# Hawkeye-FineGrained/Hawkeye

Hardware: AMD Instinct MI355X
Metric: images/sec (train fwd+bwd) BCNN VGG-16 448^2 bs64 (higher is better)
Workload: dtype f32; 1 GPU; BCNN_S2: VGG-16 448x448, per-GPU batch 64, 200 classes, SGD momentum 0.9, CE label_smoothing 0.1, full train step; global_batch=64, parallelism=dp1, memory_format=channels_last

## Files before the change

### hawkeye_amd/csrc/conv_fwd.hip

```cpp
#include "hk_common.h"
#include "hk_split_bf16.h"
#include <hk_mfma_bf16.h>
#include "../../include/hawkeye_hip.h"

namespace hk {

constexpr int CF_CO = 64;
constexpr int CF_R = 4;
constexpr int CF_SW = 32;
constexpr int CF_CK = 32;
constexpr int CF_PIX = 80;
constexpr int CF_HW = CF_SW + 2;
constexpr int CF_HPIX = (CF_R + 2) * CF_HW;
constexpr int CF_XPLANE = CF_HPIX * CF_PIX;
constexpr int CF_WPLANE = CF_CO * CF_PIX;
constexpr int CF_WTAP = 3 * CF_WPLANE;
constexpr int CF_LDS = 3 * CF_XPLANE + 2 * CF_WTAP;
constexpr int CF_XF4 = CF_HPIX * (CF_CK / 4);
constexpr int CF_XU = (CF_XF4 + 255) / 256;
constexpr int CF_FLUSH = 3;

constexpr int CF_MF_32 = 0, CF_MF_16 = 1;
constexpr int CF16_PIX = 64;
constexpr int CF16_XPLANE = CF_HPIX * CF16_PIX;
constexpr int CF16_WPLANE = CF_CO * CF16_PIX;
constexpr int CF16_WTAP = 3 * CF16_WPLANE;
constexpr int CF16_LDS = 3 * CF16_XPLANE + 2 * CF16_WTAP;
__host__ __device__ constexpr int cf16_off(int row, int kg) { return row * CF16_PIX + ((kg ^ ((row >> 1) & 2)) << 4); }
constexpr int CF_B128_GROUPS[4][16] = {{0, 1, 2, 3, 12, 13, 14, 15, 20, 21, 22, 23, 24, 25, 26, 27},
                                       {4, 5, 6, 7, 8, 9, 10, 11, 16, 17, 18, 19, 28, 29, 30, 31},
                                       {32, 33, 34, 35, 44, 45, 46, 47, 52, 53, 54, 55, 56, 57, 58, 59},
                                       {36, 37, 38, 39, 40, 41, 42, 43, 48, 49, 50, 51, 60, 61, 62, 63}};
constexpr bool cf16_group_conflict_free(int g) {
    for (int base = 0; base + 16 <= CF_HPIX; ++base) {
        unsigned seen = 0;
        for (int i = 0; i < 16; ++i) {
            const int lane = CF_B128_GROUPS[g][i], slot = (cf16_off(base + (lane & 15), lane >> 4) >> 4) & 15;
            if ((seen >> slot) & 1u) return false;
            seen |= 1u << slot;
        }
    }
    return true;
}
static_assert(cf16_group_conflict_free(0) && cf16_group_conflict_free(1) && cf16_group_conflict_free(2) && cf16_group_conflict_free(3),
              "every ds_read_b128 lane group of a CF_MF_16 fragment reads 16 different slots");
static_assert(cf16_off(16, 1) == cf16_off(0, 1) + 16 * CF16_PIX && cf16_off(35, 2) == cf16_off(3, 2) + 32 * CF16_PIX,
              "rows 16 and 32 further on are a constant offset away");
static_assert(CF16_WTAP <= CF_WTAP && CF16_WTAP == 3 * 256 * 16, "the workspace holds either image; a weight tile is three loads a thread");

template <int MF>
__global__ __launch_bounds__(256) void conv3x3_wsplit_kernel(const float* __restrict__ w, char* __restrict__ ws, int M, int K,
                                                             int transposed, long long total) {
    const long long i = (long long)blockIdx.x * 256 + threadIdx.x;
    if (i >= total) return;
    const int nchunk = K / CF_CK;
    constexpr int NQ = MF == CF_MF_32 ? 10 : 8;
    const int q = (int)(i % NQ);
    long long r = i / NQ;
    const int co = (int)(r % CF_CO);
    r /= CF_CO;
    const int tap = (int)(r % 9);
    const int chunk = (int)((r / 9) % nchunk), cot = (int)((r / 9) / nchunk);
    const long long m = (long long)cot * CF_CO + co, k0 = (long long)chunk * CF_CK + 4 * q;
    f32x4 v = {0.f, 0.f, 0.f, 0.f};
    if (q < 8) {
        if (!transposed) {
            v = *reinterpret_cast<const f32x4*>(w + (m * 9 + tap) * K + k0);
        } else {
#pragma unroll
            for (int e = 0; e < 4; ++e) v[e] = w[((k0 + e) * 9 + (8 - tap)) * M + m];
        }
    }
    bf16x4 p[3];
    wrs_split(v, p);
    if (MF == CF_MF_32) {
        char* d = ws + (size_t)r * CF_WTAP + co * CF_PIX + q * 8;
#pragma unroll
        for (int s = 0; s < 3; ++s) *reinterpret_cast<bf16x4*>(d + s * CF_WPLANE) = p[s];
    } else {
        char* d = ws + (size_t)r * CF16_WTAP + cf16_off(co, q >> 1) + (q & 1) * 8;
#pragma unroll
        for (int s = 0; s < 3; ++s) *reinterpret_cast<bf16x4*>(d + s * CF16_WPLANE) = p[s];
    }
}

__device__ __forceinline__ bf16x8 cf_frag(const char* p) {
#if defined(__HIP_DEVICE_COMPILE__)
    return *(const __attribute__((address_space(3))) bf16x8*)p;
#else
    bf16x8 f;
    __builtin_memcpy(&f, p, 16);
    return f;
#endif
}

constexpr int CF_EPI_NONE = 0, CF_EPI_RELU = 1, CF_EPI_POOL = 2, CF_EPI_MASK = 3;
constexpr int CF_PARK = CF_CO + 4;
constexpr int CF_DB_RPG = 128;
static_assert(CF_R * CF_SW * CF_PARK * 4 <= CF_LDS, "the parked tile fits the LDS of the main loop");

__device__ __forceinline__ f32x4 cf_relu4(f32x4 v) {
    f32x4 r;
#pragma unroll
    for (int t = 0; t < 4; ++t) r[t] = v[t] < 0.f ? 0.f : v[t];
    return r;
}
__device__ __forceinline__ unsigned cf_sign4(f32x4 r) {
    return (!(r[0] <= 0.f) ? 1u : 0u) | (!(r[1] <= 0.f) ? 2u : 0u) | (!(r[2] <= 0.f) ? 4u : 0u) | (!(r[3] <= 0.f) ? 8u : 0u);
}

template <int EPI>
__device__ __forceinline__ void cf16_epilogue(const f32x4 (&acc4)[4][2], const f32x4 (&sum4)[4][2], float* ldsf, float* __restrict__ y, int H,
                                              int W, int Cout, long long n, int r0, int c0, int cot, int tile, int wave, int tid, int l15,
                                              int kg, const float* __restrict__ bias, uint8_t* __restrict__ mk,
                                              double* __restrict__ part) {
    const int row = r0 + wave, c4 = Cout / 4;
    bool live[2];
    long long pix[2];
    f32x4 v[4][2];
#pragma unroll
    for (int pb = 0; pb < 2; ++pb) {
        const int col = c0 + 16 * pb + l15;
        live[pb] = row < H && col < W;
        pix[pb] = (n * H + row) * W + col;
#pragma unroll
        for (int cb = 0; cb < 4; ++cb) v[cb][pb] = sum4[cb][pb] + acc4[cb][pb];
    }
    if (EPI == CF_EPI_RELU || EPI == CF_EPI_POOL) {
        const f32x4* b4 = reinterpret_cast<const f32x4*>(bias + cot * CF_CO + 4 * kg);
#pragma unroll
        for (int cb = 0; cb < 4; ++cb) {
            const f32x4 b = b4[4 * cb];
#pragma unroll
            for (int pb = 0; pb < 2; ++pb) v[cb][pb] = cf_relu4(v[cb][pb] + b);
        }
    }
    if (EPI == CF_EPI_MASK) {
        typedef unsigned u32x4 __attribute__((ext_vector_type(4)));
#pragma unroll
        for (int pb = 0; pb < 2; ++pb) {
            u32x4 mb = {0u, 0u, 0u, 0u};
            if (live[pb]) mb = *reinterpret_cast<const u32x4*>(mk + pix[pb] * c4 + cot * (CF_CO / 4));
#pragma unroll
            for (int cb = 0; cb < 4; ++cb) {
                const unsigned bits = mb[cb] >> (8 * kg);
#pragma unroll
                for (int e = 0; e < 4; ++e) v[cb][pb][e] = ((bits >> e) & 1u) != 0u ? v[cb][pb][e] : 0.f;
            }
        }
    }
    if (EPI != CF_EPI_POOL) {
#pragma unroll
        for (int pb = 0; pb < 2; ++pb)
            if (live[pb]) {
                float* yp = y + pix[pb] * Cout + cot * CF_CO + 4 * kg;
#pragma unroll
                for (int cb = 0; cb < 4; ++cb) *reinterpret_cast<f32x4*>(yp + 16 * cb) = v[cb][pb];
            }
    }
    if (EPI == CF_EPI_RELU) {
        if (mk) {
#pragma unroll
            for (int pb = 0; pb < 2; ++pb) {
                unsigned own = 0;
#pragma unroll
                for (int cb = 0; cb < 4; ++cb) own |= cf_sign4(v[cb][pb]) << (8 * cb);
                unsigned m4 = 0;
#pragma unroll
                for (int j = 0; j < 4; ++j) m4 |= ((__shfl(own, l15 + 16 * j) >> (8 * kg)) & 0xffu) << (8 * j);
                if (live[pb]) *reinterpret_cast<unsigned*>(mk + pix[pb] * c4 + cot * (CF_CO / 4) + 4 * kg) = m4;
            }
        }
    }
    if (EPI == CF_EPI_POOL) {
        float* park = ldsf;
#pragma unroll
        for (int pb = 0; pb < 2; ++pb) {
            float* mine = park + (wave * CF_SW + 16 * pb + l15) * CF_PARK + 4 * kg;
#pragma unroll
            for (int cb = 0; cb < 4; ++cb) *reinterpret_cast<f32x4*>(mine + 16 * cb) = v[cb][pb];
        }
    }
    if (EPI == CF_EPI_MASK) {
        double s[16];
#pragma unroll
        for (int cb = 0; cb < 4; ++cb)
#pragma unroll
            for (int e = 0; e < 4; ++e) s[4 * cb + e] = (double)v[cb][0][e] + (double)v[cb][1][e];
#pragma unroll
        for (int d = 8; d >= 1; d >>= 1) {
            const bool up = (l15 & d) != 0;
#pragma unroll
            for (int i = 0; i < d; ++i) {
                const double send = up ? s[i] : s[i + d], keep = up ? s[i + d] : s[i];
                s[i] = keep + __shfl_xor(send, d);
            }
        }
        double* red = reinterpret_cast<double*>(ldsf);
        red[wave * CF_CO + 16 * (l15 >> 2) + 4 * kg + (l15 & 3)] = s[0];
        __syncthreads();
        if (tid < CF_CO)
            part[(long long)tile * Cout + cot * CF_CO + tid] = ((red[tid] + red[CF_CO + tid]) + red[2 * CF_CO + tid]) + red[3 * CF_CO + tid];
    }
}

template <int EPI, int MF>
__global__ __launch_bounds__(256, 2) void conv3x3_split_kernel(const float* __restrict__ x, const char* __restrict__ ws,
                                                               float* __restrict__ y, int H, int W, int Cin, int Cout, int nstrips,
                                                               int nrb, int ntiles, const float* __restrict__ bias,
                                                               uint8_t* __restrict__ mk, double* __restrict__ part) {
    constexpr bool M32 = MF == CF_MF_32;
    constexpr int XPLANE = M32 ? CF_XPLANE : CF16_XPLANE, WTAP = M32 ? CF_WTAP : CF16_WTAP;
    HK_DYN_LDS16(ldsf);
    char* xs = reinterpret_cast<char*>(ldsf);
    char* wb = xs + 3 * XPLANE;
    const int tid = threadIdx.x, lane = tid & 63, l31 = lane & 31, hf = lane >> 5;
    const int l15 = lane & 15, kg = lane >> 4;
    const int wave = __builtin_amdgcn_readfirstlane(tid >> 6);
    const int ncot = Cout / CF_CO, nchunk = Cin / CF_CK, total = nchunk * 9;
    int tile, cot;
    if (!xcd_map(blockIdx.x, ntiles, ncot, tile, cot)) return;
    const int strip = tile % nstrips, tr = tile / nstrips;
    const int rb = tr % nrb;
    const long long n = tr / nrb;
    const int c0 = strip * CF_SW, r0 = rb * CF_R;
    const float* xi = x + n * H * W * Cin;
    const char* wt = ws + (size_t)cot * total * WTAP + tid * 16;

    long long xoff[CF_XU];
    unsigned xok = 0;
#pragma unroll
    for (int u = 0; u < CF_XU; ++u) {
        const int idx = tid + 256 * u;
        const bool in = idx < CF_XF4;
        const int p = in ? idx >> 3 : 0, hr = p / CF_HW, hc = p - hr * CF_HW;
        const int row = r0 - 1 + hr, col = c0 - 1 + hc;
        if (in && row >= 0 && row < H && col >= 0 && col < W) xok |= 1u << u;
        const int rc = row < 0 ? 0 : (row < H ? row : H - 1), cc = col < 0 ? 0 : (col < W ? col : W - 1);
        xoff[u] = ((long long)rc * W + cc) * Cin + 4 * (idx & 7);
    }
    const int xdst = M32 ? (tid >> 3) * CF_PIX + (tid & 7) * 8 : cf16_off(tid >> 3, (tid & 7) >> 1) + (tid & 1) * 8;
    const int w3 = tid < 192 ? 3 * 4096 : 0;
    constexpr int NVW = M32 ? 4 : 3;

    f32x4 vx[CF_XU], vw[NVW];
    auto load_x = [&](int chunk) {
        const float* b = xi + chunk * CF_CK;
#pragma unroll
        for (int u = 0; u < CF_XU; ++u) HK_LOAD16_ASYNC(vx[u], b + xoff[u]);
    };
    auto load_w = [&](int it) {
        const char* b = wt + (size_t)it * WTAP;
#pragma unroll
        for (int u = 0; u < 3; ++u) HK_LOAD16_ASYNC(vw[u], reinterpret_cast<const float*>(b + 4096 * u));
        if constexpr (M32) {
            HK_LOAD16_ASYNC(vw[3], reinterpret_cast<const float*>(b + w3));
        }
    };
    auto store_x = [&]() {
        const f32x4 zero = {0.f, 0.f, 0.f, 0.f};
#pragma unroll
        for (int u = 0; u < CF_XU; ++u) {
            if (tid + 256 * u < CF_XF4) {
                bf16x4 p[3];
                wrs_split(((xok >> u) & 1) ? vx[u] : zero, p);
#pragma unroll
                for (int s = 0; s < 3; ++s) *reinterpret_cast<bf16x4*>(xs + s * XPLANE + xdst + u * 32 * (M32 ? CF_PIX : CF16_PIX)) = p[s];
            }
        }
    };
    auto store_w = [&](int buf) {
        char* d = wb + buf * WTAP + tid * 16;
#pragma unroll
        for (int u = 0; u < 3; ++u) *reinterpret_cast<f32x4*>(d + 4096 * u) = vw[u];
        if constexpr (M32) {
            if (tid < 192) *reinterpret_cast<f32x4*>(d + 3 * 4096) = vw[3];
        }
    };

    f32x16 acc[2], sum[2];
    f32x4 acc4[4][2], sum4[4][2];
    if constexpr (M32) {
#pragma unroll
        for (int cb = 0; cb < 2; ++cb)
#pragma unroll
            for (int i = 0; i < 16; ++i) acc[cb][i] = sum[cb][i] = 0.f;
    } else {
#pragma unroll
        for (int cb = 0; cb < 4; ++cb)
#pragma unroll
            for (int pb = 0; pb < 2; ++pb)
#pragma unroll
                for (int e = 0; e < 4; ++e) acc4[cb][pb][e] = sum4[cb][pb][e] = 0.f;
    }

    load_w(0);
    load_x(0);
    __builtin_amdgcn_s_waitcnt(HK_VMCNT_IMM(0));
#pragma unroll
    for (int u = 0; u < NVW; ++u) HK_PIN_LOADED(vw[u]);
#pragma unroll
    for (int u = 0; u < CF_XU; ++u) HK_PIN_LOADED(vx[u]);
    store_x();
    store_w(0);
    __syncthreads();

    const int aoff = l31 * CF_PIX + hf * 16;
    const int boff = (wave * CF_HW + l31) * CF_PIX + hf * 16;
    int since = 0;
    for (int chunk = 0; chunk < nchunk; ++chunk) {
        const bool more = chunk + 1 < nchunk;
#pragma unroll
        for (int tap = 0; tap < 9; ++tap) {
            const int it = chunk * 9 + tap;
            load_w(it + 1 < total ? it + 1 : it);
            if (tap == 5) load_x(more ? chunk + 1 : chunk);
            if constexpr (M32) {
            const char* A = wb + (it & 1) * CF_WTAP + aoff;
            const char* B = xs + boff + ((tap / 3) * CF_HW + tap % 3) * CF_PIX;
            bf16x8 a[2][2][3], b[2][3];
#pragma unroll
            for (int ks = 0; ks < 2; ++ks)
#pragma unroll
                for (int s = 0; s < 3; ++s) {
                    b[ks][s] = cf_frag(B + s * CF_XPLANE + ks * 32);
                    a[ks][0][s] = cf_frag(A + s * CF_WPLANE + ks * 32);
                    a[ks][1][s] = cf_frag(A + s * CF_WPLANE + 32 * CF_PIX + ks * 32);
                }
#pragma unroll
            for (int ks = 0; ks < 2; ++ks)
#pragma unroll
                for (int cb = 0; cb < 2; ++cb) {
                    acc[cb] = __builtin_amdgcn_mfma_f32_32x32x16_bf16(a[ks][cb][1], b[ks][1], acc[cb], 0, 0, 0);
                    acc[cb] = __builtin_amdgcn_mfma_f32_32x32x16_bf16(a[ks][cb][0], b[ks][2], acc[cb], 0, 0, 0);
                    acc[cb] = __builtin_amdgcn_mfma_f32_32x32x16_bf16(a[ks][cb][2], b[ks][0], acc[cb], 0, 0, 0);
                    acc[cb] = __builtin_amdgcn_mfma_f32_32x32x16_bf16(a[ks][cb][0], b[ks][1], acc[cb], 0, 0, 0);
                    acc[cb] = __builtin_amdgcn_mfma_f32_32x32x16_bf16(a[ks][cb][1], b[ks][0], acc[cb], 0, 0, 0);
                    acc[cb] = __builtin_amdgcn_mfma_f32_32x32x16_bf16(a[ks][cb][0], b[ks][0], acc[cb], 0, 0, 0);
                }
            } else {
                const char* A = wb + (it & 1) * CF16_WTAP + cf16_off(l15, kg);
                const char* B = xs + cf16_off(wave * CF_HW + l15 + (tap / 3) * CF_HW + tap % 3, kg);
                bf16x8 a[4][3], b[2][3];
#pragma unroll
                for (int s = 0; s < 3; ++s) {
#pragma unroll
                    for (int pb = 0; pb < 2; ++pb) b[pb][s] = cf_frag(B + s * CF16_XPLANE + pb * 16 * CF16_PIX);
#pragma unroll
                    for (int cb = 0; cb < 4; ++cb) a[cb][s] = cf_frag(A + s * CF16_WPLANE + cb * 16 * CF16_PIX);
                }
                constexpr int PA[6] = {1, 0, 2, 0, 1, 0}, PB[6] = {1, 2, 0, 1, 0, 0};
#pragma unroll
                for (int pr = 0; pr < 6; ++pr)
#pragma unroll
                    for (int cb = 0; cb < 4; ++cb)
#pragma unroll
                        for (int pb = 0; pb < 2; ++pb) acc4[cb][pb] = mfma_f32_16x16x32_bf16(a[cb][PA[pr]], b[pb][PB[pr]], acc4[cb][pb]);
            }
            if (tap == 5) __builtin_amdgcn_s_waitcnt(HK_VMCNT_IMM(CF_XU));
            else __builtin_amdgcn_s_waitcnt(HK_VMCNT_IMM(0));
#pragma unroll
            for (int u = 0; u < NVW; ++u) HK_PIN_LOADED(vw[u]);
            if (tap == 6) {
#pragma unroll
                for (int u = 0; u < CF_XU; ++u) HK_PIN_LOADED(vx[u]);
            }
            store_w((it + 1) & 1);
            if (tap == 8 && more) {
                __syncthreads();
                store_x();
            }
            __syncthreads();
        }
        if (++since == CF_FLUSH) {
            if constexpr (M32) {
#pragma unroll
                for (int cb = 0; cb < 2; ++cb) {
                    sum[cb] += acc[cb];
#pragma unroll
                    for (int i = 0; i < 16; ++i) acc[cb][i] = 0.f;
                }
            } else {
#pragma unroll
                for (int cb = 0; cb < 4; ++cb)
#pragma unroll
                    for (int pb = 0; pb < 2; ++pb) {
                        sum4[cb][pb] += acc4[cb][pb];
#pragma unroll
                        for (int e = 0; e < 4; ++e) acc4[cb][pb][e] = 0.f;
                    }
            }
            since = 0;
        }
    }
    if constexpr (!M32) {
        cf16_epilogue<EPI>(acc4, sum4, ldsf, y, H, W, Cout, n, r0, c0, cot, tile, wave, tid, l15, kg, bias, mk, part);
        if (EPI != CF_EPI_POOL) return;
    }
    const int row = r0 + wave, col = c0 + l31;
    if (EPI == CF_EPI_NONE) {
        if (row < H && col < W) {
            float* yp = y + ((n * H + row) * W + col) * Cout + cot * CF_CO + 4 * hf;
#pragma unroll
            for (int cb = 0; cb < 2; ++cb)
#pragma unroll
                for (int j = 0; j < 4; ++j) {
                    f32x4 v;
#pragma unroll
                    for (int e = 0; e < 4; ++e) v[e] = sum[cb][4 * j + e] + acc[cb][4 * j + e];
                    *reinterpret_cast<f32x4*>(yp + cb * 32 + 8 * j) = v;
                }
        }
        return;
    }
    const bool live = row < H && col < W;
    const long long pix = (n * H + row) * W + col;
    const int c4 = Cout / 4;
    f32x4 v[2][4];
    if constexpr (M32) {
#pragma unroll
    for (int cb = 0; cb < 2; ++cb)
#pragma unroll
        for (int j = 0; j < 4; ++j)
#pragma unroll
            for (int e = 0; e < 4; ++e) v[cb][j][e] = sum[cb][4 * j + e] + acc[cb][4 * j + e];
    }
    if (M32 && (EPI == CF_EPI_RELU || EPI == CF_EPI_POOL)) {
        const f32x4* b4 = reinterpret_cast<const f32x4*>(bias + cot * CF_CO + 4 * hf);
#pragma unroll
        for (int cb = 0; cb < 2; ++cb)
#pragma unroll
            for (int j = 0; j < 4; ++j) v[cb][j] = cf_relu4(v[cb][j] + b4[8 * cb + 2 * j]);
    }
    if (EPI == CF_EPI_RELU) {
        if (live) {
            float* yp = y + pix * Cout + cot * CF_CO + 4 * hf;
#pragma unroll
            for (int cb = 0; cb < 2; ++cb)
#pragma unroll
                for (int j = 0; j < 4; ++j) *reinterpret_cast<f32x4*>(yp + cb * 32 + 8 * j) = v[cb][j];
        }
        if (mk) {
            unsigned own[2];
#pragma unroll
            for (int cb = 0; cb < 2; ++cb) {
                own[cb] = 0;
#pragma unroll
                for (int j = 0; j < 4; ++j) own[cb] |= cf_sign4(v[cb][j]) << (8 * j);
            }
            const unsigned theirs0 = __shfl_xor(own[0], 32), theirs1 = __shfl_xor(own[1], 32);
            const unsigned ev = hf ? theirs1 : own[0], od = hf ? own[1] : theirs0;
            unsigned long long m8 = 0;
#pragma unroll
            for (int k = 0; k < 4; ++k)
                m8 |= ((unsigned long long)((ev >> (8 * k)) & 0xffu) << (16 * k)) | ((unsigned long long)((od >> (8 * k)) & 0xffu) << (16 * k + 8));
            if (live) *reinterpret_cast<unsigned long long*>(mk + pix * c4 + cot * (CF_CO / 4) + 8 * hf) = m8;
        }
    }
    if (EPI == CF_EPI_POOL) {
        float* park = ldsf;
        if constexpr (M32) {
        float* mine = park + (wave * CF_SW + l31) * CF_PARK + 4 * hf;
#pragma unroll
        for (int cb = 0; cb < 2; ++cb)
#pragma unroll
            for (int j = 0; j < 4; ++j) *reinterpret_cast<f32x4*>(mine + cb * 32 + 8 * j) = v[cb][j];
        }
        __syncthreads();
        const int q = tid & 15, pc = tid >> 4;
        const int Ho = H / 2, Wo = W / 2;
#pragma unroll
        for (int u = 0; u < 2; ++u) {
            const float* src = park + (2 * u * CF_SW + 2 * pc) * CF_PARK + 4 * q;
            f32x4 m = *reinterpret_cast<const f32x4*>(src);
            unsigned code = 0;
#pragma unroll
            for (int k = 1; k < 4; ++k) {
                const f32x4 a = *reinterpret_cast<const f32x4*>(src + ((k >> 1) * CF_SW + (k & 1)) * CF_PARK);
#pragma unroll
                for (int t = 0; t < 4; ++t) {
                    const bool take = (a[t] > m[t]) || (a[t] != a[t]);
                    m[t] = take ? a[t] : m[t];
                    code = take ? ((code & ~(3u << (2 * t))) | ((unsigned)k << (2 * t))) : code;
                }
            }
            unsigned t1 = __shfl_xor(code, 1);
            unsigned c2 = (q & 1) ? (t1 | (code << 8)) : (code | (t1 << 8));
            unsigned t2 = __shfl_xor(c2, 2);
            unsigned c4b = (q & 2) ? (t2 | (c2 << 16)) : (c2 | (t2 << 16));
            unsigned t4 = __shfl_xor(c4b, 4);
            const unsigned long long lo = (q & 4) ? t4 : c4b, hi = (q & 4) ? c4b : t4;
            const int ho = r0 / 2 + u, wo = c0 / 2 + pc;
            if (ho < Ho && wo < Wo) {
                const long long opix = (n * Ho + ho) * Wo + wo;
                *reinterpret_cast<f32x4*>(y + opix * Cout + cot * CF_CO + 4 * q) = m;
                if ((q & 7) == 0) *reinterpret_cast<unsigned long long*>(mk + opix * c4 + cot * (CF_CO / 4) + q) = lo | (hi << 32);
            }
        }
    }
    if (EPI == CF_EPI_MASK) {
        typedef unsigned u32x4 __attribute__((ext_vector_type(4)));
        u32x4 mb = {0u, 0u, 0u, 0u};
        if (live) mb = *reinterpret_cast<const u32x4*>(mk + pix * c4 + cot * (CF_CO / 4));
        double s[32];
#pragma unroll
        for (int cb = 0; cb < 2; ++cb)
#pragma unroll
            for (int j = 0; j < 4; ++j) {
                const unsigned bits = mb[2 * cb + (j >> 1)] >> (8 * (2 * (j & 1) + hf));
#pragma unroll
                for (int e = 0; e < 4; ++e) {
                    v[cb][j][e] = ((bits >> e) & 1u) != 0u ? v[cb][j][e] : 0.f;
                    s[16 * cb + 4 * j + e] = v[cb][j][e];
                }
            }
        if (live) {
            float* yp = y + pix * Cout + cot * CF_CO + 4 * hf;
#pragma unroll
            for (int cb = 0; cb < 2; ++cb)
#pragma unroll
                for (int j = 0; j < 4; ++j) *reinterpret_cast<f32x4*>(yp + cb * 32 + 8 * j) = v[cb][j];
        }
#pragma unroll
        for (int d = 16; d >= 1; d >>= 1) {
            const bool up = (l31 & d) != 0;
#pragma unroll
            for (int i = 0; i < d; ++i) {
                const double send = up ? s[i] : s[i + d], keep = up ? s[i + d] : s[i];
                s[i] = keep + __shfl_xor(send, d);
            }
        }
        double* red = reinterpret_cast<double*>(ldsf);
        red[wave * CF_CO + 32 * (l31 >> 4) + 8 * ((l31 >> 2) & 3) + 4 * hf + (l31 & 3)] = s[0];
        __syncthreads();
        if (tid < CF_CO)
            part[(long long)tile * Cout + cot * CF_CO + tid] = ((red[tid] + red[CF_CO + tid]) + red[2 * CF_CO + tid]) + red[3 * CF_CO + tid];
    }
}

template <int Q, typename OUT>
__global__ __launch_bounds__(64 * Q) void conv3x3_colsum_kernel(const double* __restrict__ part, int nrows, int nel, int rpg,
                                                                OUT* __restrict__ out) {
    __shared__ double red[Q][64];
    const int l = threadIdx.x & 63, q = threadIdx.x >> 6;
    const int e = blockIdx.x * 64 + l;
    const int beg = blockIdx.y * rpg, end = beg + rpg < nrows ? beg + rpg : nrows;
    double s = 0.0;
    if (e < nel) {
        int k = beg + q;
        for (; k + 7 * Q < end; k += 8 * Q) {
            double t[8];
#pragma unroll
            for (int u = 0; u < 8; ++u) t[u] = part[(long long)(k + Q * u) * nel + e];
#pragma unroll
            for (int u = 0; u < 8; ++u) s += t[u];
        }
        for (; k < end; k += Q) s += part[(long long)k * nel + e];
    }
    red[q][l] = s;
    __syncthreads();
    if (q == 0 && e < nel) {
        double t = red[0][l];
        for (int k = 1; k < Q; ++k) t += red[k][l];
        out[(long long)blockIdx.y * nel + e] = (OUT)t;
    }
}

template <int EPI, int MF>
static int conv3x3_run_on(const float* x, const float* w, float* y, int N, int H, int W, int K, int M, bool transposed, void* ws,
                          hipStream_t stream, const float* bias, uint8_t* mk, double* part) {
    constexpr int LDS = MF == CF_MF_32 ? CF_LDS : CF16_LDS;
    const long long nstrips = ((long long)W + CF_SW - 1) / CF_SW, nrb = ((long long)H + CF_R - 1) / CF_R, ntiles = N * nrb * nstrips;
    const int ncot = M / CF_CO;
    if ((ntiles + NXCD) * ncot > 0x7fffffffll) return HK_ERR_UNSUPPORTED;
    const long long total = (long long)ncot * (K / CF_CK) * 9 * CF_CO * (MF == CF_MF_32 ? 10 : 8);
    hipLaunchKernelGGL(conv3x3_wsplit_kernel<MF>, dim3((unsigned)((total + 255) / 256)), dim3(256), 0, stream, w, (char*)ws, M, K,
                       transposed ? 1 : 0, total);
    HK_LAUNCH_CHECK();
    HK_ALLOW_BIG_LDS((conv3x3_split_kernel<EPI, MF>), LDS);
    hipLaunchKernelGGL((conv3x3_split_kernel<EPI, MF>), dim3((unsigned)xcd_grid((int)ntiles, ncot)), dim3(256), LDS, stream, x, (const char*)ws,
                       y, H, W, K, M, (int)nstrips, (int)nrb, (int)ntiles, bias, mk, part);
    HK_LAUNCH_CHECK();
    return HK_OK;
}
template <int EPI>
static int conv3x3_run(const float* x, const float* w, float* y, int N, int H, int W, int K, int M, bool transposed, void* ws,
                       hipStream_t stream, const float* bias = nullptr, uint8_t* mk = nullptr, double* part = nullptr) {
    if (tuning().conv_mfma == 1) return conv3x3_run_on<EPI, CF_MF_16>(x, w, y, N, H, W, K, M, transposed, ws, stream, bias, mk, part);
    return conv3x3_run_on<EPI, CF_MF_32>(x, w, y, N, H, W, K, M, transposed, ws, stream, bias, mk, part);
}

static int conv3x3_check(const float* x, const float* w, float* y, int N, int H, int W, int Cin, int Cout, void* ws, size_t ws_bytes,
                         int knob) {
    if (!x || !w || !y || N <= 0 || H <= 0 || W <= 0 || Cin <= 0 || Cout <= 0) return HK_ERR_BAD_ARG;
    if (!ws || ws_bytes < hk_conv3x3_ws_bytes(Cin, Cout)) return HK_ERR_WORKSPACE;
    if (Cin % 64 != 0 || Cout % 64 != 0 || (long long)Cout * 9 * Cin > 0x7fffffffll || !aligned16(x) || !aligned16(w) || !aligned16(y) ||
        !aligned16(ws) || knob == 0)
        return HK_ERR_UNSUPPORTED;
    return HK_OK;
}

static long long conv3x3_tiles(int N, int H, int W) {
    return (long long)N * (((long long)H + CF_R - 1) / CF_R) * (((long long)W + CF_SW - 1) / CF_SW);
}
static long long conv3x3_groups(long long ntiles) { return ntiles > CF_DB_RPG ? (ntiles + CF_DB_RPG - 1) / CF_DB_RPG : 0; }

}

using namespace hk;

extern "C" size_t hk_conv3x3_ws_bytes(int Cin, int Cout) {
    if (Cin <= 0 || Cout <= 0) return 0;
    const size_t a = ((size_t)Cout + 63) / 64 * (((size_t)Cin + 31) / 32), b = ((size_t)Cin + 63) / 64 * (((size_t)Cout + 31) / 32);
    return (a > b ? a : b) * 9 * CF_WTAP;
}

extern "C" int hk_conv3x3_fwd(const float* x, const float* w, float* y, int N, int H, int W, int Cin, int Cout, void* ws, size_t ws_bytes,
                              hk_stream_t stream) {
    const int rc = conv3x3_check(x, w, y, N, H, W, Cin, Cout, ws, ws_bytes, tuning().conv_fwd);
    return rc != HK_OK ? rc : conv3x3_run<CF_EPI_NONE>(x, w, y, N, H, W, Cin, Cout, false, ws, (hipStream_t)stream);
}

extern "C" int hk_conv3x3_bwd_data(const float* dy, const float* w, float* dx, int N, int H, int W, int Cin, int Cout, void* ws,
                                   size_t ws_bytes, hk_stream_t stream) {
    const int rc = conv3x3_check(dy, w, dx, N, H, W, Cin, Cout, ws, ws_bytes, tuning().conv_bwd_data);
    return rc != HK_OK ? rc : conv3x3_run<CF_EPI_NONE>(dy, w, dx, N, H, W, Cout, Cin, true, ws, (hipStream_t)stream);
}

extern "C" int hk_conv3x3_bias_relu_fwd(const float* x, const float* w, const float* bias, float* y, uint8_t* mask, int N, int H, int W,
                                        int Cin, int Cout, void* ws, size_t ws_bytes, hk_stream_t stream) {
    if (!bias) return HK_ERR_BAD_ARG;
    const int rc = conv3x3_check(x, w, y, N, H, W, Cin, Cout, ws, ws_bytes, tuning().conv_fwd);
    if (rc != HK_OK) return rc;
    if (!aligned16(bias) || (((uintptr_t)mask) & 7) != 0 || tuning().conv_epi < 1) return HK_ERR_UNSUPPORTED;
    return conv3x3_run<CF_EPI_RELU>(x, w, y, N, H, W, Cin, Cout, false, ws, (hipStream_t)stream, bias, mask);
}

extern "C" int hk_conv3x3_bias_relu_pool_fwd(const float* x, const float* w, const float* bias, float* p, uint8_t* argmax, int N, int H,
                                             int W, int Cin, int Cout, void* ws, size_t ws_bytes, hk_stream_t stream) {
    if (!bias || !argmax) return HK_ERR_BAD_ARG;
    const int rc = conv3x3_check(x, w, p, N, H, W, Cin, Cout, ws, ws_bytes, tuning().conv_fwd);
    if (rc != HK_OK) return rc;
    if (H % 2 != 0 || W % 2 != 0 || !aligned16(bias) || (((uintptr_t)argmax) & 7) != 0 || tuning().conv_epi < 1) return HK_ERR_UNSUPPORTED;
    return conv3x3_run<CF_EPI_POOL>(x, w, p, N, H, W, Cin, Cout, false, ws, (hipStream_t)stream, bias, argmax);
}

extern "C" size_t hk_conv3x3_masked_ws_bytes(int N, int H, int W, int Cin, int Cout) {
    if (N <= 0 || H <= 0 || W <= 0 || Cin <= 0 || Cout <= 0) return 0;
    const long long ntiles = conv3x3_tiles(N, H, W);
    return hk_conv3x3_ws_bytes(Cin, Cout) + (size_t)(ntiles + conv3x3_groups(ntiles)) * Cin * sizeof(double);
}

extern "C" int hk_conv3x3_masked_bwd_data(const float* dy, const float* w, const uint8_t* mask, float* dx, float* dbias, int N, int H, int W,
                                          int Cin, int Cout, void* ws, size_t ws_bytes, hk_stream_t stream) {
    if (!mask || !dbias) return HK_ERR_BAD_ARG;
    const int rc = conv3x3_check(dy, w, dx, N, H, W, Cin, Cout, ws, ws_bytes, tuning().conv_bwd_data);
    if (rc != HK_OK) return rc;
    if (ws_bytes < hk_conv3x3_masked_ws_bytes(N, H, W, Cin, Cout)) return HK_ERR_WORKSPACE;
    if (!aligned16(mask) || tuning().conv_epi < 2) return HK_ERR_UNSUPPORTED;
    const long long ntiles = conv3x3_tiles(N, H, W), ngroups = conv3x3_groups(ntiles);
    if (ntiles > 0x7fffffffll || ngroups > 65535) return HK_ERR_UNSUPPORTED;
    double* part = reinterpret_cast<double*>((char*)ws + hk_conv3x3_ws_bytes(Cin, Cout));
    double* grp = part + ntiles * Cin;
    const int rc2 = conv3x3_run<CF_EPI_MASK>(dy, w, dx, N, H, W, Cout, Cin, true, ws, (hipStream_t)stream, nullptr, const_cast<uint8_t*>(mask), part);
    if (rc2 != HK_OK) return rc2;
    const dim3 cols((unsigned)(Cin / 64));
    if (ngroups > 0) {
        hipLaunchKernelGGL((conv3x3_colsum_kernel<16, double>), dim3(cols.x, (unsigned)ngroups), dim3(1024), 0, (hipStream_t)stream,
                           (const double*)part, (int)ntiles, Cin, CF_DB_RPG, grp);
        HK_LAUNCH_CHECK();
        hipLaunchKernelGGL((conv3x3_colsum_kernel<16, float>), cols, dim3(1024), 0, (hipStream_t)stream, (const double*)grp, (int)ngroups, Cin,
                           (int)ngroups, dbias);
    } else {
        hipLaunchKernelGGL((conv3x3_colsum_kernel<16, float>), cols, dim3(1024), 0, (hipStream_t)stream, (const double*)part, (int)ntiles, Cin,
                           (int)ntiles, dbias);
    }
    HK_LAUNCH_CHECK();
    return HK_OK;
}
```

Before: 566.7 images/sec.

## Stage conv-forward weights with direct global-to-LDS loads and merge tap barriers

```diff
diff --git a/hawkeye_amd/csrc/conv_fwd.hip b/hawkeye_amd/csrc/conv_fwd.hip
--- a/hawkeye_amd/csrc/conv_fwd.hip
+++ b/hawkeye_amd/csrc/conv_fwd.hip
@@ -26,6 +26,13 @@
 constexpr int CF16_WPLANE = CF_CO * CF16_PIX;
 constexpr int CF16_WTAP = 3 * CF16_WPLANE;
 constexpr int CF16_LDS = 3 * CF16_XPLANE + 2 * CF16_WTAP;
+#define CF_TAP_BARRIER(n)                                                                                      \
+    do {                                                                                                       \
+        asm volatile("" ::: "memory");                                         \
+        __builtin_amdgcn_s_waitcnt(HK_VMCNT_IMM(n) & ~(15 << 8));                                              \
+        __builtin_amdgcn_s_barrier();                                                                          \
+        asm volatile("" ::: "memory");                                                                         \
+    } while (0)
 __host__ __device__ constexpr int cf16_off(int row, int kg) { return row * CF16_PIX + ((kg ^ ((row >> 1) & 2)) << 4); }
 constexpr int CF_B128_GROUPS[4][16] = {{0, 1, 2, 3, 12, 13, 14, 15, 20, 21, 22, 23, 24, 25, 26, 27},
                                        {4, 5, 6, 7, 8, 9, 10, 11, 16, 17, 18, 19, 28, 29, 30, 31},
@@ -240,21 +247,20 @@
         xoff[u] = ((long long)rc * W + cc) * Cin + 4 * (idx & 7);
     }
     const int xdst = M32 ? (tid >> 3) * CF_PIX + (tid & 7) * 8 : cf16_off(tid >> 3, (tid & 7) >> 1) + (tid & 1) * 8;
-    const int w3 = tid < 192 ? 3 * 4096 : 0;
-    constexpr int NVW = M32 ? 4 : 3;
-
-    f32x4 vx[CF_XU], vw[NVW];
+
+    f32x4 vx[CF_XU];
     auto load_x = [&](int chunk) {
         const float* b = xi + chunk * CF_CK;
 #pragma unroll
         for (int u = 0; u < CF_XU; ++u) HK_LOAD16_ASYNC(vx[u], b + xoff[u]);
     };
-    auto load_w = [&](int it) {
+    auto load_w = [&](int it, int buf) {
         const char* b = wt + (size_t)it * WTAP;
-#pragma unroll
-        for (int u = 0; u < 3; ++u) HK_LOAD16_ASYNC(vw[u], reinterpret_cast<const float*>(b + 4096 * u));
+        char* d = wb + buf * WTAP + wave * 1024;
+#pragma unroll
+        for (int u = 0; u < 3; ++u) glds16(reinterpret_cast<const float*>(b + 4096 * u), reinterpret_cast<float*>(d + 4096 * u));
         if constexpr (M32) {
-            HK_LOAD16_ASYNC(vw[3], reinterpret_cast<const float*>(b + w3));
+            if (wave < 3) glds16(reinterpret_cast<const float*>(b + 3 * 4096), reinterpret_cast<float*>(d + 3 * 4096));
         }
     };
     auto store_x = [&]() {
@@ -269,14 +275,6 @@
             }
         }
     };
-    auto store_w = [&](int buf) {
-        char* d = wb + buf * WTAP + tid * 16;
-#pragma unroll
-        for (int u = 0; u < 3; ++u) *reinterpret_cast<f32x4*>(d + 4096 * u) = vw[u];
-        if constexpr (M32) {
-            if (tid < 192) *reinterpret_cast<f32x4*>(d + 3 * 4096) = vw[3];
-        }
-    };
 
     f32x16 acc[2], sum[2];
     f32x4 acc4[4][2], sum4[4][2];
@@ -294,16 +292,13 @@
                 for (int e = 0; e < 4; ++e) acc4[cb][pb][e] = sum4[cb][pb][e] = 0.f;
     }
 
-    load_w(0);
+    load_w(0, 0);
     load_x(0);
     __builtin_amdgcn_s_waitcnt(HK_VMCNT_IMM(0));
 #pragma unroll
-    for (int u = 0; u < NVW; ++u) HK_PIN_LOADED(vw[u]);
-#pragma unroll
     for (int u = 0; u < CF_XU; ++u) HK_PIN_LOADED(vx[u]);
     store_x();
-    store_w(0);
-    __syncthreads();
+    HK_LDS_BARRIER();
 
     const int aoff = l31 * CF_PIX + hf * 16;
     const int boff = (wave * CF_HW + l31) * CF_PIX + hf * 16;
@@ -313,7 +308,7 @@
 #pragma unroll
         for (int tap = 0; tap < 9; ++tap) {
             const int it = chunk * 9 + tap;
-            load_w(it + 1 < total ? it + 1 : it);
+            load_w(it + 1 < total ? it + 1 : it, (it + 1) & 1);
             if (tap == 5) load_x(more ? chunk + 1 : chunk);
             if constexpr (M32) {
             const char* A = wb + (it & 1) * CF_WTAP + aoff;
@@ -327,6 +322,7 @@
                     a[ks][0][s] = cf_frag(A + s * CF_WPLANE + ks * 32);
                     a[ks][1][s] = cf_frag(A + s * CF_WPLANE + 32 * CF_PIX + ks * 32);
                 }
+            __builtin_amdgcn_sched_barrier(0);
 #pragma unroll
             for (int ks = 0; ks < 2; ++ks)
 #pragma unroll
@@ -349,6 +345,7 @@
 #pragma unroll
                     for (int cb = 0; cb < 4; ++cb) a[cb][s] = cf_frag(A + s * CF16_WPLANE + cb * 16 * CF16_PIX);
                 }
+                __builtin_amdgcn_sched_barrier(0);
                 constexpr int PA[6] = {1, 0, 2, 0, 1, 0}, PB[6] = {1, 2, 0, 1, 0, 0};
 #pragma unroll
                 for (int pr = 0; pr < 6; ++pr)
@@ -357,20 +354,16 @@
 #pragma unroll
                         for (int pb = 0; pb < 2; ++pb) acc4[cb][pb] = mfma_f32_16x16x32_bf16(a[cb][PA[pr]], b[pb][PB[pr]], acc4[cb][pb]);
             }
-            if (tap == 5) __builtin_amdgcn_s_waitcnt(HK_VMCNT_IMM(CF_XU));
-            else __builtin_amdgcn_s_waitcnt(HK_VMCNT_IMM(0));
-#pragma unroll
-            for (int u = 0; u < NVW; ++u) HK_PIN_LOADED(vw[u]);
+            if (tap == 5) CF_TAP_BARRIER(CF_XU);
+            else CF_TAP_BARRIER(0);
             if (tap == 6) {
 #pragma unroll
                 for (int u = 0; u < CF_XU; ++u) HK_PIN_LOADED(vx[u]);
             }
-            store_w((it + 1) & 1);
             if (tap == 8 && more) {
-                __syncthreads();
                 store_x();
-            }
-            __syncthreads();
+                HK_LDS_BARRIER();
+            }
         }
         if (++since == CF_FLUSH) {
             if constexpr (M32) {
```

Result: faster. 580.5 images/sec, median of 6 (+2.4%).
